# tj12323/GeoPurify

Hardware: AMD Instinct MI355X
Metric: scenes/sec (ScanNet-val shape) + pooled-feature GB/s vs HBM peak (higher is better)
Workload: dtype f32 (student convolutions and pooling: f16 hi/lo split operands, 3 MFMAs per product, fp32 accumulate)

## Files before the change

### geopurify_amd/csrc/knn.hip

```cpp
#include "gp_grid.h"

namespace {

constexpr int KNN_MAXSEL = 128;
constexpr int KNN_MAXTIE = 256;

template <int R>
struct KnnCfg {
    static constexpr int B = (8 * R + 1) * (8 * R + 1);
    static constexpr int HB = (B + 63) / 64 * 64;
};

constexpr int KNN_KEEP = 32;
constexpr int KNN_KEEP_ROW_BITS = 25;

template <int R, int WAVES, bool KEEP = false>
__global__ void __launch_bounds__(WAVES * 64)
knn_ring_kernel(const void *grid, const int32_t *__restrict__ coords, const int32_t *__restrict__ ids, int64_t nv,
                int k, int32_t *__restrict__ nbr, const int32_t *__restrict__ qlist,
                const int32_t *__restrict__ qcount, int32_t *__restrict__ fail_list, int32_t *__restrict__ fail_count) {
    constexpr int B = KnnCfg<R>::B, HB = KnnCfg<R>::HB;
    __shared__ int s_hist[WAVES][HB];
    __shared__ unsigned long long s_selkey[WAVES][KNN_MAXSEL];
    __shared__ int s_selrow[WAVES][KNN_MAXSEL];
    __shared__ int s_tieid[WAVES][KNN_MAXTIE];
    __shared__ int s_tierow[WAVES][KNN_MAXTIE];
    __shared__ int s_cnt[WAVES][2];
    __shared__ int s_cstart[WAVES][(2 * R + 1) * (2 * R + 1) * (2 * R + 1)], s_coff[WAVES][(2 * R + 1) * (2 * R + 1) * (2 * R + 1) + 1];

    const int wv = threadIdx.x >> 6, lane = threadIdx.x & 63;
    int64_t widx = (int64_t)blockIdx.x * WAVES + wv;
    int64_t total = qlist ? (int64_t)*qcount : nv;
    if (widx >= total) return;
    const int qi = __builtin_amdgcn_readfirstlane(qlist ? qlist[widx] : (int)widx);
    GpGridView g(grid);
    const int qx = coords[(int64_t)qi * 3], qy = coords[(int64_t)qi * 3 + 1], qz = coords[(int64_t)qi * 3 + 2];
    const int cx0 = (qx - g.h->origin[0]) >> 3, cy0 = (qy - g.h->origin[1]) >> 3, cz0 = (qz - g.h->origin[2]) >> 3;
    int *hist = s_hist[wv];
    for (int b = lane; b < HB; b += 64) hist[b] = 0;
    if (lane < 2) s_cnt[wv][lane] = 0;
    constexpr int SIDE = 2 * R + 1, NC = SIDE * SIDE * SIDE;
    int *cstart = s_cstart[wv], *coff = s_coff[wv];
    int total_c = 0;
    for (int c0 = 0; c0 < NC; c0 += 64) {
        const int c = c0 + lane;
        int start = 0, cnt = 0;
        if (c < NC) {
            const int dx = c % SIDE - R, dy = (c / SIDE) % SIDE - R, dz = c / (SIDE * SIDE) - R;
            const int slot = g.cell_slot(cx0 + dx, cy0 + dy, cz0 + dz);
            if (slot >= 0) { start = g.recs[slot].start; cnt = g.recs[slot].count; }
        }
        int incl = cnt;
#pragma unroll
        for (int o = 1; o < 64; o <<= 1) {
            int t = __shfl_up(incl, o, 64);
            if (lane >= o) incl += t;
        }
        if (c < NC) { cstart[c] = start; coff[c] = total_c + incl - cnt; }
        total_c += __shfl(incl, 63, 64);
    }
    if (lane == 0) coff[NC] = total_c;
    gp_wave_sync();
    auto row_of = [&](int j) {
        int lo = 0, hi = NC - 1;
        while (lo < hi) {
            const int mid = (lo + hi + 1) >> 1;
            if (coff[mid] <= j) lo = mid; else hi = mid - 1;
        }
        return cstart[lo] + (j - coff[lo]);
    };

    static_assert(!KEEP || KnnCfg<R>::B <= 127, "a kept candidate holds d^2 in 7 bits");
    const bool kept = KEEP && total_c <= 64 * KNN_KEEP;
    unsigned keep[KEEP ? KNN_KEEP : 1];
    if constexpr (KEEP) {
        if (kept) {
#pragma unroll
            for (int i = 0; i < KNN_KEEP; i += 2) {
                if (i * 64 < total_c) {
                    const int ja = i * 64 + lane, jb = ja + 64;
                    const bool va = ja < total_c, vb = jb < total_c;
                    const int64_t ra = va ? row_of(ja) : 0, rb = vb ? row_of(jb) : 0;
                    const int ax = coords[ra * 3], ay = coords[ra * 3 + 1], az = coords[ra * 3 + 2];
                    const int bx = coords[rb * 3], by = coords[rb * 3 + 1], bz = coords[rb * 3 + 2];
                    const int da = (ax - qx) * (ax - qx) + (ay - qy) * (ay - qy) + (az - qz) * (az - qz);
                    const int db = (bx - qx) * (bx - qx) + (by - qy) * (by - qy) + (bz - qz) * (bz - qz);
                    if (va && da < B) atomicAdd(&hist[da], 1);
                    if (vb && db < B) atomicAdd(&hist[db], 1);
                    keep[i] = ((unsigned)(va ? min(da, 127) : 127) << KNN_KEEP_ROW_BITS) | (unsigned)ra;
                    keep[i + 1] = ((unsigned)(vb ? min(db, 127) : 127) << KNN_KEEP_ROW_BITS) | (unsigned)rb;
                }
            }
        }
    }
    for (int j0 = kept ? total_c : 0; j0 < total_c; j0 += 128) {
        const int ja = j0 + lane, jb = j0 + 64 + lane;
        const bool va = ja < total_c, vb = jb < total_c;
        const int64_t ra = va ? row_of(ja) : 0, rb = vb ? row_of(jb) : 0;
        const int ax = coords[ra * 3], ay = coords[ra * 3 + 1], az = coords[ra * 3 + 2];
        const int bx = coords[rb * 3], by = coords[rb * 3 + 1], bz = coords[rb * 3 + 2];
        const int da = (ax - qx) * (ax - qx) + (ay - qy) * (ay - qy) + (az - qz) * (az - qz);
        const int db = (bx - qx) * (bx - qx) + (by - qy) * (by - qy) + (bz - qz) * (bz - qz);
        if (va && da < B) atomicAdd(&hist[da], 1);
        if (vb && db < B) atomicAdd(&hist[db], 1);
    }
    gp_wave_sync();

    constexpr int CH = HB / 64;
    int loc = 0;
#pragma unroll
    for (int c = 0; c < CH; ++c) loc += hist[lane * CH + c];
    int incl = loc;
#pragma unroll
    for (int o = 1; o < 64; o <<= 1) {
        int t = __shfl_up(incl, o, 64);
        if (lane >= o) incl += t;
    }
    int tot = __shfl(incl, 63, 64);
    const int need = k + 1;
    bool fail = tot < need;
    int T = 0, c_lt = 0;
    if (!fail) {
        int excl = incl - loc;
        unsigned long long m = __ballot(incl >= need);
        int owner = __ffsll((long long)m) - 1;
        int myT = 0, mylt = 0;
        if (lane == owner) {
            int run = excl;
            for (int c = 0; c < CH; ++c) {
                int h = hist[lane * CH + c];
                if (run + h >= need) { myT = lane * CH + c; mylt = run; break; }
                run += h;
            }
        }
        T = __shfl(myT, owner, 64);
        c_lt = __shfl(mylt, owner, 64);
        if (hist[T] > KNN_MAXTIE) fail = true;
    }
    if (fail) {
        if (lane == 0) {
            int p = atomicAdd(fail_count, 1);
            fail_list[p] = qi;
        }
        return;
    }

    auto emit = [&](int64_t r, int d2) {
        if (d2 < T) {
            int id = ids ? ids[r] : (int)r;
            int p = atomicAdd(&s_cnt[wv][0], 1);
            s_selkey[wv][p] = ((unsigned long long)(unsigned)d2 << 32) | (unsigned)id;
            s_selrow[wv][p] = (int)r;
        } else if (d2 == T) {
            int id = ids ? ids[r] : (int)r;
            int p = atomicAdd(&s_cnt[wv][1], 1);
            s_tieid[wv][p] = id;
            s_tierow[wv][p] = (int)r;
        }
    };
    if constexpr (KEEP) {
        if (kept) {
#pragma unroll
            for (int i = 0; i < KNN_KEEP; ++i)
                if (i * 64 < total_c) emit((int64_t)(keep[i] & ((1u << KNN_KEEP_ROW_BITS) - 1u)), (int)(keep[i] >> KNN_KEEP_ROW_BITS));
        }
    }
    for (int j0 = kept ? total_c : 0; j0 < total_c; j0 += 64) {
        const int j = j0 + lane;
        if (j < total_c) {
            const int64_t r = row_of(j);
            int ex = coords[r * 3] - qx, ey = coords[r * 3 + 1] - qy, ez = coords[r * 3 + 2] - qz;
            emit(r, ex * ex + ey * ey + ez * ez);
        }
    }
    gp_wave_sync();
    const int m_tie = s_cnt[wv][1];
    const int take = need - c_lt;
    for (int t = lane; t < m_tie; t += 64) {
        int id = s_tieid[wv][t];
        int rank = 0;
        for (int u = 0; u < m_tie; ++u) rank += (s_tieid[wv][u] < id);
        if (rank < take) {
            s_selkey[wv][c_lt + rank] = ((unsigned long long)(unsigned)T << 32) | (unsigned)id;
            s_selrow[wv][c_lt + rank] = s_tierow[wv][t];
        }
    }
    gp_wave_sync();

    for (int t = lane; t < need; t += 64) {
        unsigned long long key = s_selkey[wv][t];
        int rank = 0;
        for (int u = 0; u < need; ++u) rank += (s_selkey[wv][u] < key);
        if (rank > 0) nbr[(int64_t)qi * k + rank - 1] = s_selrow[wv][t];
    }
}

__global__ void __launch_bounds__(256)
knn_exhaustive_kernel(const int32_t *__restrict__ coords, const int32_t *__restrict__ ids, int64_t nv, int k,
                      int32_t *__restrict__ nbr, const int32_t *__restrict__ qlist, const int32_t *__restrict__ qcount) {
    __shared__ int s_red[4];
    __shared__ unsigned long long s_selkey[KNN_MAXSEL];
    __shared__ int s_selrow[KNN_MAXSEL];
    __shared__ int s_n;
    const int total = *qcount;
    for (int w = blockIdx.x; w < total; w += gridDim.x) {
        const int qi = qlist[w];
        const int qx = coords[(int64_t)qi * 3], qy = coords[(int64_t)qi * 3 + 1], qz = coords[(int64_t)qi * 3 + 2];
        const int need = k + 1;
        auto keyof = [&](int64_t r) {
            long long ex = coords[r * 3] - qx, ey = coords[r * 3 + 1] - qy, ez = coords[r * 3 + 2] - qz;
            unsigned long long d2 = (unsigned long long)(ex * ex + ey * ey + ez * ez);
            unsigned id = (unsigned)(ids ? ids[r] : (int)r);
            return (d2 << 32) | id;
        };
        unsigned long long lo = 0, hi = ~0ull;
        while (lo < hi) {
            unsigned long long mid = lo + ((hi - lo) >> 1);
            int c = 0;
            for (int64_t r = threadIdx.x; r < nv; r += 256) c += (keyof(r) <= mid);
            c = gp_wave_sum_i(c);
            __syncthreads();
            if ((threadIdx.x & 63) == 0) s_red[threadIdx.x >> 6] = c;
            __syncthreads();
            int tot = s_red[0] + s_red[1] + s_red[2] + s_red[3];
            if (tot >= need) hi = mid; else lo = mid + 1;
        }
        if (threadIdx.x == 0) s_n = 0;
        __syncthreads();
        for (int64_t r = threadIdx.x; r < nv; r += 256) {
            unsigned long long key = keyof(r);
            if (key <= lo) {
                int p = atomicAdd(&s_n, 1);
                if (p < KNN_MAXSEL) { s_selkey[p] = key; s_selrow[p] = (int)r; }
            }
        }
        __syncthreads();
        for (int t = threadIdx.x; t < need; t += 256) {
            unsigned long long key = s_selkey[t];
            int rank = 0;
            for (int u = 0; u < need; ++u) rank += (s_selkey[u] < key);
            if (rank > 0) nbr[(int64_t)qi * k + rank - 1] = s_selrow[t];
        }
        __syncthreads();
    }
}

__global__ void zero2_kernel(int32_t *a, int32_t *b) {
    if (threadIdx.x == 0) { *a = 0; *b = 0; }
}

}

extern "C" size_t gp_knn_workspace_bytes(int64_t nv) {
    GpCarver cv(nullptr, 0);
    cv.take<int32_t>(64);
    cv.take<int32_t>(nv);
    cv.take<int32_t>(nv);
    return cv.off;
}

static int knn_lattice(bool read_once, const void *grid, const int32_t *coords, const int32_t *ids, int64_t nv, int32_t k,
                       int32_t *nbr, void *workspace, size_t workspace_bytes, void *stream_) {
    GP_CHECK_ARG(grid && coords && nbr && workspace, "gp_knn_lattice: null argument");
    GP_CHECK_ARG(k >= 1 && k <= GP_KNN_MAX_K, "gp_knn_lattice: k=%d not in 1..%d", k, GP_KNN_MAX_K);
    GP_CHECK_ARG(nv > k, "gp_knn_lattice: need more than k voxels (nv=%lld, k=%d)", (long long)nv, k);
    GpCarver cv(workspace, workspace_bytes);
    int32_t *counts = cv.take<int32_t>(64);
    int32_t *list_a = cv.take<int32_t>(nv);
    int32_t *list_b = cv.take<int32_t>(nv);
    if (!cv.ok()) { gp_set_error("gp_knn_lattice: workspace too small (%zu < %zu)", workspace_bytes, cv.off); return GP_ENOMEM; }
    hipStream_t s = gp_stream(stream_);
    zero2_kernel<<<1, 64, 0, s>>>(counts, counts + 1);
    constexpr int W1 = 4, W3 = 2;
    if (read_once && nv <= ((int64_t)1 << KNN_KEEP_ROW_BITS))
        knn_ring_kernel<1, W1, true><<<(int)((nv + W1 - 1) / W1), W1 * 64, 0, s>>>(grid, coords, ids, nv, k, nbr, nullptr, nullptr,
                                                                                list_a, counts);
    else
        knn_ring_kernel<1, W1><<<(int)((nv + W1 - 1) / W1), W1 * 64, 0, s>>>(grid, coords, ids, nv, k, nbr, nullptr, nullptr,
                                                                          list_a, counts);
    knn_ring_kernel<3, W3><<<(int)((nv + W3 - 1) / W3), W3 * 64, 0, s>>>(grid, coords, ids, nv, k, nbr, list_a, counts,
                                                                      list_b, counts + 1);
    knn_exhaustive_kernel<<<1024, 256, 0, s>>>(coords, ids, nv, k, nbr, list_b, counts + 1);
    GP_CHECK_LAUNCH();
    return GP_OK;
}

extern "C" int gp_knn_lattice(const void *grid, const int32_t *coords, const int32_t *ids, int64_t nv, int32_t k,
                              int32_t *nbr, void *workspace, size_t workspace_bytes, void *stream_) {
    return knn_lattice(true, grid, coords, ids, nv, k, nbr, workspace, workspace_bytes, stream_);
}

extern "C" int gp_knn_lattice_two_pass(const void *grid, const int32_t *coords, const int32_t *ids, int64_t nv, int32_t k,
                                       int32_t *nbr, void *workspace, size_t workspace_bytes, void *stream_) {
    return knn_lattice(false, grid, coords, ids, nv, k, nbr, workspace, workspace_bytes, stream_);
}
```

Before: 46.85.

## Use histogram cursors for KNN selection and grid-stride the radius-3 fallback pass

For the read-once radius-1 path, the distance histogram is turned into exclusive-prefix cursors. Selected neighbours are then scattered into runs ordered by distance, so the final ranking only compares within equal-distance runs instead of running an O(need²) comparison over all keys. Separately, the radius-3 fallback kernel now launches a capped grid (2048 workgroups) and grid-strides over the fail list, rather than launching one wave per voxel when only a few queries fail. The helpers are factored out. The capped grid could limit parallelism when the fail list is large.

```diff
diff --git a/geopurify_amd/csrc/knn.hip b/geopurify_amd/csrc/knn.hip
--- a/geopurify_amd/csrc/knn.hip
+++ b/geopurify_amd/csrc/knn.hip
@@ -14,11 +14,131 @@
 constexpr int KNN_KEEP = 32;
 constexpr int KNN_KEEP_ROW_BITS = 25;
 
-template <int R, int WAVES, bool KEEP = false>
-__global__ void __launch_bounds__(WAVES * 64)
-knn_ring_kernel(const void *grid, const int32_t *__restrict__ coords, const int32_t *__restrict__ ids, int64_t nv,
-                int k, int32_t *__restrict__ nbr, const int32_t *__restrict__ qlist,
-                const int32_t *__restrict__ qcount, int32_t *__restrict__ fail_list, int32_t *__restrict__ fail_count) {
+template <int HB, bool CURSORS = false>
+__device__ __forceinline__ bool knn_threshold(int *hist, int lane, int need, int &T, int &c_lt) {
+    constexpr int CH = HB / 64;
+    int loc = 0;
+#pragma unroll
+    for (int c = 0; c < CH; ++c) loc += hist[lane * CH + c];
+    int incl = loc;
+#pragma unroll
+    for (int o = 1; o < 64; o <<= 1) {
+        int t = __shfl_up(incl, o, 64);
+        if (lane >= o) incl += t;
+    }
+    int tot = __shfl(incl, 63, 64);
+    if (tot < need) return false;
+    int excl = incl - loc;
+    unsigned long long m = __ballot(incl >= need);
+    int owner = __ffsll((long long)m) - 1;
+    int myT = 0, mylt = 0;
+    if (lane == owner) {
+        int run = excl;
+        for (int c = 0; c < CH; ++c) {
+            int h = hist[lane * CH + c];
+            if (run + h >= need) { myT = lane * CH + c; mylt = run; break; }
+            run += h;
+        }
+    }
+    T = __shfl(myT, owner, 64);
+    c_lt = __shfl(mylt, owner, 64);
+    if (hist[T] > KNN_MAXTIE) return false;
+    if constexpr (CURSORS) {
+        gp_wave_sync();
+        int run = excl;
+#pragma unroll
+        for (int c = 0; c < CH; ++c) {
+            const int h = hist[lane * CH + c];
+            hist[lane * CH + c] = run;
+            run += h;
+        }
+        gp_wave_sync();
+    }
+    return true;
+}
+
+__device__ __forceinline__ void knn_emit(const int32_t *__restrict__ ids, int64_t r, int d2, int T, unsigned long long *selkey,
+                                         int *selrow, int *tieid, int *tierow, int *cnt) {
+    if (d2 < T) {
+        int id = ids ? ids[r] : (int)r;
+        int p = atomicAdd(&cnt[0], 1);
+        selkey[p] = ((unsigned long long)(unsigned)d2 << 32) | (unsigned)id;
+        selrow[p] = (int)r;
+    } else if (d2 == T) {
+        int id = ids ? ids[r] : (int)r;
+        int p = atomicAdd(&cnt[1], 1);
+        tieid[p] = id;
+        tierow[p] = (int)r;
+    }
+}
+
+__device__ __forceinline__ void knn_rank_store(int lane, int need, int T, int c_lt, unsigned long long *selkey, int *selrow,
+                                               const int *tieid, const int *tierow, const int *cnt, int32_t *__restrict__ nbr_row) {
+    gp_wave_sync();
+    const int m_tie = cnt[1];
+    const int take = need - c_lt;
+    for (int t = lane; t < m_tie; t += 64) {
+        int id = tieid[t];
+        int rank = 0;
+        for (int u = 0; u < m_tie; ++u) rank += (tieid[u] < id);
+        if (rank < take) {
+            selkey[c_lt + rank] = ((unsigned long long)(unsigned)T << 32) | (unsigned)id;
+            selrow[c_lt + rank] = tierow[t];
+        }
+    }
+    gp_wave_sync();
+    for (int t = lane; t < need; t += 64) {
+        unsigned long long key = selkey[t];
+        int rank = 0;
+        for (int u = 0; u < need; ++u) rank += (selkey[u] < key);
+        if (rank > 0) nbr_row[rank - 1] = selrow[t];
+    }
+}
+
+__device__ __forceinline__ void knn_emit_run(int id, int r, int d2, int T, int *hist, unsigned long long *selkey, int *selrow,
+                                             int *tieid, int *tierow, int *ntie) {
+    if (d2 < T) {
+        const int p = atomicAdd(&hist[d2], 1);
+        selkey[p] = ((unsigned long long)(unsigned)d2 << 32) | (unsigned)id;
+        selrow[p] = r;
+    } else if (d2 == T) {
+        const int p = atomicAdd(ntie, 1);
+        tieid[p] = id;
+        tierow[p] = r;
+    }
+}
+__device__ __forceinline__ void knn_rank_store_runs(int lane, int need, int c_lt, const int *hist, const unsigned long long *selkey,
+                                                    const int *selrow, const int *tieid, const int *tierow, int m_tie,
+                                                    int32_t *__restrict__ nbr_row) {
+    const int take = need - c_lt;
+    for (int t = lane; t < m_tie; t += 64) {
+        const int id = tieid[t];
+        int rank = 0;
+        for (int u = 0; u < m_tie; ++u) rank += (tieid[u] < id);
+        if (rank < take && c_lt + rank > 0) nbr_row[c_lt + rank - 1] = tierow[t];
+    }
+    for (int t = lane; t < c_lt; t += 64) {
+        const unsigned long long key = selkey[t];
+        const int d2 = (int)(key >> 32);
+        const unsigned id = (unsigned)key;
+        const int lo = d2 ? hist[d2 - 1] : 0, hi = hist[d2];
+        int rank = lo;
+        for (int u = lo; u < hi; ++u) rank += ((unsigned)selkey[u] < id);
+        if (rank > 0) nbr_row[rank - 1] = selrow[t];
+    }
+}
+
+__device__ __forceinline__ void knn_fail(int lane, int qi, int32_t *__restrict__ fail_list, int32_t *__restrict__ fail_count) {
+    if (lane == 0) {
+        int p = atomicAdd(fail_count, 1);
+        fail_list[p] = qi;
+    }
+}
+
+template <int R, int WAVES, bool KEEP>
+__device__ __forceinline__ void knn_ring_query(const void *grid, const int32_t *__restrict__ coords, const int32_t *__restrict__ ids,
+                                               int k, int32_t *__restrict__ nbr, const int qi, int32_t *__restrict__ fail_list,
+                                               int32_t *__restrict__ fail_count) {
     constexpr int B = KnnCfg<R>::B, HB = KnnCfg<R>::HB;
     __shared__ int s_hist[WAVES][HB];
     __shared__ unsigned long long s_selkey[WAVES][KNN_MAXSEL];
@@ -29,10 +149,6 @@
     __shared__ int s_cstart[WAVES][(2 * R + 1) * (2 * R + 1) * (2 * R + 1)], s_coff[WAVES][(2 * R + 1) * (2 * R + 1) * (2 * R + 1) + 1];
 
     const int wv = threadIdx.x >> 6, lane = threadIdx.x & 63;
-    int64_t widx = (int64_t)blockIdx.x * WAVES + wv;
-    int64_t total = qlist ? (int64_t)*qcount : nv;
-    if (widx >= total) return;
-    const int qi = __builtin_amdgcn_readfirstlane(qlist ? qlist[widx] : (int)widx);
     GpGridView g(grid);
     const int qx = coords[(int64_t)qi * 3], qy = coords[(int64_t)qi * 3 + 1], qz = coords[(int64_t)qi * 3 + 2];
     const int cx0 = (qx - g.h->origin[0]) >> 3, cy0 = (qy - g.h->origin[1]) >> 3, cz0 = (qz - g.h->origin[2]) >> 3;
@@ -106,56 +222,20 @@
     }
     gp_wave_sync();
 
-    constexpr int CH = HB / 64;
-    int loc = 0;
-#pragma unroll
-    for (int c = 0; c < CH; ++c) loc += hist[lane * CH + c];
-    int incl = loc;
-#pragma unroll
-    for (int o = 1; o < 64; o <<= 1) {
-        int t = __shfl_up(incl, o, 64);
-        if (lane >= o) incl += t;
-    }
-    int tot = __shfl(incl, 63, 64);
     const int need = k + 1;
-    bool fail = tot < need;
     int T = 0, c_lt = 0;
-    if (!fail) {
-        int excl = incl - loc;
-        unsigned long long m = __ballot(incl >= need);
-        int owner = __ffsll((long long)m) - 1;
-        int myT = 0, mylt = 0;
-        if (lane == owner) {
-            int run = excl;
-            for (int c = 0; c < CH; ++c) {
-                int h = hist[lane * CH + c];
-                if (run + h >= need) { myT = lane * CH + c; mylt = run; break; }
-                run += h;
-            }
-        }
-        T = __shfl(myT, owner, 64);
-        c_lt = __shfl(mylt, owner, 64);
-        if (hist[T] > KNN_MAXTIE) fail = true;
-    }
-    if (fail) {
-        if (lane == 0) {
-            int p = atomicAdd(fail_count, 1);
-            fail_list[p] = qi;
-        }
+    constexpr bool RUNS = KEEP;
+    if (!knn_threshold<HB, RUNS>(hist, lane, need, T, c_lt)) {
+        knn_fail(lane, qi, fail_list, fail_count);
         return;
     }
 
     auto emit = [&](int64_t r, int d2) {
-        if (d2 < T) {
-            int id = ids ? ids[r] : (int)r;
-            int p = atomicAdd(&s_cnt[wv][0], 1);
-            s_selkey[wv][p] = ((unsigned long long)(unsigned)d2 << 32) | (unsigned)id;
-            s_selrow[wv][p] = (int)r;
-        } else if (d2 == T) {
-            int id = ids ? ids[r] : (int)r;
-            int p = atomicAdd(&s_cnt[wv][1], 1);
-            s_tieid[wv][p] = id;
-            s_tierow[wv][p] = (int)r;
+        if constexpr (RUNS) {
+            if (d2 <= T)
+                knn_emit_run(ids ? ids[r] : (int)r, (int)r, d2, T, hist, s_selkey[wv], s_selrow[wv], s_tieid[wv], s_tierow[wv], &s_cnt[wv][1]);
+        } else {
+            knn_emit(ids, r, d2, T, s_selkey[wv], s_selrow[wv], s_tieid[wv], s_tierow[wv], s_cnt[wv]);
         }
     };
     if constexpr (KEEP) {
@@ -173,25 +253,27 @@
             emit(r, ex * ex + ey * ey + ez * ez);
         }
     }
-    gp_wave_sync();
-    const int m_tie = s_cnt[wv][1];
-    const int take = need - c_lt;
-    for (int t = lane; t < m_tie; t += 64) {
-        int id = s_tieid[wv][t];
-        int rank = 0;
-        for (int u = 0; u < m_tie; ++u) rank += (s_tieid[wv][u] < id);
-        if (rank < take) {
-            s_selkey[wv][c_lt + rank] = ((unsigned long long)(unsigned)T << 32) | (unsigned)id;
-            s_selrow[wv][c_lt + rank] = s_tierow[wv][t];
-        }
-    }
-    gp_wave_sync();
-
-    for (int t = lane; t < need; t += 64) {
-        unsigned long long key = s_selkey[wv][t];
-        int rank = 0;
-        for (int u = 0; u < need; ++u) rank += (s_selkey[wv][u] < key);
-        if (rank > 0) nbr[(int64_t)qi * k + rank - 1] = s_selrow[wv][t];
+    if constexpr (RUNS) {
+        gp_wave_sync();
+        knn_rank_store_runs(lane, need, c_lt, hist, s_selkey[wv], s_selrow[wv], s_tieid[wv], s_tierow[wv], s_cnt[wv][1],
+                            nbr + (int64_t)qi * k);
+    } else {
+        knn_rank_store(lane, need, T, c_lt, s_selkey[wv], s_selrow[wv], s_tieid[wv], s_tierow[wv], s_cnt[wv], nbr + (int64_t)qi * k);
+    }
+}
+
+template <int R, int WAVES, bool KEEP = false, bool STRIDE = false>
+__global__ void __launch_bounds__(WAVES * 64)
+knn_ring_kernel(const void *grid, const int32_t *__restrict__ coords, const int32_t *__restrict__ ids, int64_t nv,
+                int k, int32_t *__restrict__ nbr, const int32_t *__restrict__ qlist,
+                const int32_t *__restrict__ qcount, int32_t *__restrict__ fail_list, int32_t *__restrict__ fail_count) {
+    const int wv = threadIdx.x >> 6;
+    const int64_t total = qlist ? (int64_t)*qcount : nv;
+    for (int64_t widx = (int64_t)blockIdx.x * WAVES + wv; widx < total; widx += (int64_t)gridDim.x * WAVES) {
+        const int qi = __builtin_amdgcn_readfirstlane(qlist ? qlist[widx] : (int)widx);
+        knn_ring_query<R, WAVES, KEEP>(grid, coords, ids, k, nbr, qi, fail_list, fail_count);
+        if constexpr (!STRIDE) return;
+        gp_wave_sync();
     }
 }
 
@@ -272,14 +354,15 @@
     hipStream_t s = gp_stream(stream_);
     zero2_kernel<<<1, 64, 0, s>>>(counts, counts + 1);
     constexpr int W1 = 4, W3 = 2;
+    const int grid1 = (int)((nv + W1 - 1) / W1);
     if (read_once && nv <= ((int64_t)1 << KNN_KEEP_ROW_BITS))
-        knn_ring_kernel<1, W1, true><<<(int)((nv + W1 - 1) / W1), W1 * 64, 0, s>>>(grid, coords, ids, nv, k, nbr, nullptr, nullptr,
-                                                                                list_a, counts);
+        knn_ring_kernel<1, W1, true><<<grid1, W1 * 64, 0, s>>>(grid, coords, ids, nv, k, nbr, nullptr, nullptr, list_a, counts);
     else
-        knn_ring_kernel<1, W1><<<(int)((nv + W1 - 1) / W1), W1 * 64, 0, s>>>(grid, coords, ids, nv, k, nbr, nullptr, nullptr,
-                                                                          list_a, counts);
-    knn_ring_kernel<3, W3><<<(int)((nv + W3 - 1) / W3), W3 * 64, 0, s>>>(grid, coords, ids, nv, k, nbr, list_a, counts,
-                                                                      list_b, counts + 1);
+        knn_ring_kernel<1, W1><<<grid1, W1 * 64, 0, s>>>(grid, coords, ids, nv, k, nbr, nullptr, nullptr, list_a, counts);
+    constexpr int64_t RING3_WGS = 2048;
+    const int64_t wgs3 = (nv + W3 - 1) / W3;
+    knn_ring_kernel<3, W3, false, true><<<(int)(wgs3 < RING3_WGS ? wgs3 : RING3_WGS), W3 * 64, 0, s>>>(grid, coords, ids, nv, k, nbr, list_a, counts,
+                                                                                        list_b, counts + 1);
     knn_exhaustive_kernel<<<1024, 256, 0, s>>>(coords, ids, nv, k, nbr, list_b, counts + 1);
     GP_CHECK_LAUNCH();
     return GP_OK;
```

After: 46.78. No clear change (-0.1%).
